# naver/multi-hmr

Hardware: AMD Instinct MI355X
Metric: images/sec (whole node) ViT-L 896x896 bs32 (higher is better)
Workload: dtype f16; 1 GPU; multiHMR_896_L full forward: dinov2_vitl14 896x896, 32 images/GPU, 8 pinned persons/image -> HPH (depth 2) -> SMPL-X LBS; image-sharded x1; global_batch=32, parallelism=dp1 (images)

## Files before the change

multi_hmr_amd/csrc/gemm.hip:

```cpp
#include <stdlib.h>
#include "mhmr_common.h"
#include <string.h>
#include <stdlib.h>
#include "mhmr_internal.h"

namespace {

constexpr int BM = 128, BN = 128, BK = 64;
constexpr int TILE_BYTES = 128 * BK * 2;

template <int DT, int EPI>
__global__ __launch_bounds__(256, 2) void gemm_kernel(const GemmArgs g) {
    typedef typename Op<DT>::T T;
    typedef typename Op<DT>::V8 V8;
    typedef typename Op<DT>::V4 V4;
    extern __shared__ __attribute__((aligned(16))) char smem[];

    const int tid = threadIdx.x, lane = tid & 63;
    const int w = __builtin_amdgcn_readfirstlane(tid >> 6);
    const int hi = lane >> 5, l31 = lane & 31;

    const int nbn = g.N / BN;
    const int bid = xcd_remap(blockIdx.x, gridDim.x);
    const int tn = bid % nbn, tm = bid / nbn;
// ... 131 lines not shown
                    *(f32x4*)op = *(const f32x4*)op + gm * v;
                } else if constexpr (EPI == EPI_PATCH) {
                    if (m < g.Mvalid) {
                        const int b = m / g.Np, n_in = m - b * g.Np;
                        v += *(const f32x4*)(g.pos + (size_t)(1 + n_in) * g.N + n);
                        *(f32x4*)((float*)g.out + ((size_t)b * g.Tp + n_in) * g.ldo + n) = v;
                    }
                } else {
                    *(f32x4*)((float*)g.out + (size_t)m * g.ldo + n) = v;
                }
            }
        }
    } else {
        const int rpi = g.img_rows > 0 ? g.img_rows : g.Tp;
        const int b = m0 / rpi, t0 = m0 - b * rpi;
#pragma unroll
        for (int qj = 0; qj < 2; ++qj) {
            const int n = n0 + 64 * wq_ + 32 * qj + l31;
            const float bv = g.bias ? g.bias[n] : 0.f;
            const int h = n >> 6, d = n & 63;
            T* base = (T*)g.out + ((size_t)(b * g.H + h) * 64 + d) * g.Tp;
#pragma unroll
            for (int pi = 0; pi < 2; ++pi) {
#pragma unroll
                for (int rg = 0; rg < 4; ++rg) {
                    const int t = t0 + 64 * wp_ + 32 * pi + 8 * rg + 4 * hi;
                    const int ts = (t & ~12) | ((t & 4) << 1) | ((t & 8) >> 1);
                    V4 o;
#pragma unroll
                    for (int e = 0; e < 4; ++e) o[e] = (T)(acc[pi][qj][4 * rg + e] + bv);
                    *(V4*)(base + ts) = o;
                }
            }
        }
    }
}

template <int DT>
int launch_dt(const GemmArgs& g, hipStream_t s) {
    const int grid = (g.M / BM) * (g.N / BN);
    const size_t lds = 4 * TILE_BYTES;
#define MHMR_GEMM_CASE(E)                                                                                   \
    case E: {                                                                                               \
        static DeviceOnce once;                                                                             \
        int dev = 0;                                                                                        \
        const int need = once.need(&dev);                                                                   \
        if (need == -2) return MHMR_ERR_BAD_ARG;                                                            \
        if (need >= 0) {                                                                                    \
            hipError_t e = hipFuncSetAttribute((const void*)gemm_kernel<DT, E>, hipFuncAttributeMaxDynamicSharedMemorySize, \
                                               (int)lds);                                                   \
            if (e != hipSuccess) return (int)e;                                                             \
            once.mark(dev);                                                                                 \
        }                                                                                                   \
        hipLaunchKernelGGL((gemm_kernel<DT, E>), dim3(grid), dim3(256), lds, s, g);                         \
        break;                                                                                              \
    }
    switch (g.epi) {
        MHMR_GEMM_CASE(EPI_OP16)
        MHMR_GEMM_CASE(EPI_OP16_GELU)
        MHMR_GEMM_CASE(EPI_OP16_RELU)
        MHMR_GEMM_CASE(EPI_RESID)
        MHMR_GEMM_CASE(EPI_PATCH)
        MHMR_GEMM_CASE(EPI_F32)
        MHMR_GEMM_CASE(EPI_VT)
        MHMR_GEMM_CASE(EPI_OP16_QK)
        default:
            return MHMR_ERR_BAD_ARG;
    }
#undef MHMR_GEMM_CASE
    MHMR_CHECK_LAUNCH();
    return 0;
}

}

int mhmr_cu_count() {
    static std::atomic<int> cus[64];
    int dev = 0;
    if (hipGetDevice(&dev) != hipSuccess) return -1;
    if (dev >= 0 && dev < 64) {
        const int c = cus[dev].load(std::memory_order_relaxed);
        if (c > 0) return c;
    }
    hipDeviceProp_t prop;
    if (hipGetDeviceProperties(&prop, dev) != hipSuccess) return -1;
    if (dev >= 0 && dev < 64) cus[dev].store(prop.multiProcessorCount, std::memory_order_relaxed);
    return prop.multiProcessorCount;
}

namespace {
struct ColGroupEnv {
    int narrow = 2, wide = 2;
    static int lg(int v) { return v <= 0 ? 0 : v == 1 ? 2 : v == 2 ? 1 : v == 4 ? 2 : v == 8 ? 3 : v == 16 ? 4 : v == 32 ? 5 : 0; }
    ColGroupEnv() {
        const char* e = getenv("MHMR_COLGROUP");
        if (!e) return;
        narrow = wide = lg(atoi(e));
        if (const char* c = strchr(e, ',')) wide = lg(atoi(c + 1));
    }
};
}
static const bool g_force_gemm128 = getenv("MHMR_GEMM128") != nullptr;

bool mhmr_splitk_plan(int M, int N, int K, int* ksplit, int* nslices) {
    static const bool on = !(getenv("MHMR_SPLITK") && atoi(getenv("MHMR_SPLITK")) == 0);
    if (!on || g_force_gemm128 || M <= 0 || M % 256 || N % 256 || K % 128) return false;
    if (N > 1024) return false;
    const int ncu = mhmr_cu_count();
    const int tiles = (M / 256) * (N / 256), nt = K / 64;
    if (ncu <= 0 || tiles <= 0) return false;
    int S = ncu / tiles;
    if (S > 8) S = 8;
    if (S > nt / 4) S = nt / 4;
    if (S < 2) return false;
    int ks = (nt + S - 1) / S;
    ks += ks & 1;
    S = (nt + ks - 1) / ks;
    if (S < 2) return false;
    *ksplit = ks;
    *nslices = S;
    return true;
}

int mhmr_launch_gemm(const GemmArgs& g, int dtype, hipStream_t s) {
    if (g.M <= 0 || g.N <= 0 || g.K <= 0 || g.M % BM || g.N % BN || g.K % BK) return MHMR_ERR_BAD_SHAPE;
    if (g.lda % 8 || g.ldw % 8) return MHMR_ERR_BAD_SHAPE;
    if (g.epi == EPI_VT && (g.Tp % 64 || g.N % 64)) return MHMR_ERR_BAD_SHAPE;
    if (g.epi == EPI_VT && (g.img_rows > 0 ? g.img_rows : g.Tp) % BM && (g_force_gemm128 || !mhmr_gemm256_eligible(g))) return MHMR_ERR_BAD_SHAPE;
    if (g.img_rows > 0 && (g.img_rows % BM || g.M % g.img_rows || g.img_stride < g.img_rows || g.epi == EPI_PATCH)) return MHMR_ERR_BAD_SHAPE;
    if (g.a_k > 0 && !g.lo8 && (g.a_k % BK || (g.K != 2 * g.a_k && g.K != 3 * g.a_k) || g.ldw < g.K || (g.K == 3 * g.a_k && g.lda < 2 * g.a_k))) return MHMR_ERR_BAD_SHAPE;
    if (g.epi == EPI_OP16_QK && g.N % 128) return MHMR_ERR_BAD_SHAPE;
    if (g.lo8 && (g_force_gemm128 || !mhmr_gemm256_eligible(g))) return MHMR_ERR_BAD_SHAPE;
    if ((g.x8_off > 0 || g.ldx16 > 0) && !g.x16) return MHMR_ERR_BAD_ARG;
    if (g.ksplit > 0 && (g_force_gemm128 || !mhmr_gemm256_eligible(g))) return MHMR_ERR_BAD_SHAPE;
    if (g.out2 && (g_force_gemm128 || !mhmr_gemm256_eligible(g))) return MHMR_ERR_BAD_SHAPE;
    if (g.n_valid > 0 && g.n_valid != g.N && (g_force_gemm128 || !mhmr_gemm256_eligible(g))) return MHMR_ERR_BAD_SHAPE;
    if (g.x16 || g.pstats || g.rowstats) {
        if (g_force_gemm128 || !mhmr_gemm256_eligible(g)) return MHMR_ERR_BAD_SHAPE;
        if (g.rowstats && g.K < 256) return MHMR_ERR_BAD_SHAPE;
        if (g.rowstats && (g.bias || !g.colsum || !g.fbias || !(g.epi == EPI_OP16_QK || g.epi == EPI_VT || g.epi == EPI_OP16_GELU))) return MHMR_ERR_BAD_ARG;
        if ((g.x16 != nullptr) != (g.pstats != nullptr) || (g.x16 && g.epi != EPI_RESID)) return MHMR_ERR_BAD_ARG;
    }
    prof_begin(PROF_GEMM, s);
    int rc;
    if (!g_force_gemm128 && mhmr_gemm256_eligible(g)) {
        GemmArgs g2 = g;
        static const char* st = getenv("MHMR_STAGGER_PCT");
        const int pct = st ? atoi(st) : (g.img_rows > 0 ? 0 : 100);
        if (g.epi == EPI_RESID && (g.M / 256) * (g.N / 256) >= 1024 && pct > 0)
            g2.stagger_ticks = (int)((g.K / 64 * 1.4 + 18.0) * 25.0 * pct / 100.0);
        static const ColGroupEnv cge;
        const int nbn = g.N / 256;
        g2.colgroup = g.ksplit > 0 ? 0 : nbn >= 16 ? cge.wide : cge.narrow;
        if (g.img_rows > 256) g2.img_magic = (unsigned)((1ull << 32) / (unsigned)(g.img_rows >> 8)) + 1u;
        rc = mhmr_launch_gemm256(g2, dtype, s);
    }
    else rc = dtype == MHMR_DT_F16 ? launch_dt<MHMR_DT_F16>(g, s) : launch_dt<MHMR_DT_BF16>(g, s);
    prof_end(PROF_GEMM, s, 2.0 * g.M * g.N * (g.lo8 ? 2.0 * g.a_k : (double)g.K));
    return rc;
}
```

multi_hmr_amd/csrc/gemm256.hip:

```cpp
#include <type_traits>
#include "mhmr_common.h"
#include "mhmr_internal.h"

namespace {

constexpr int HT = 16384;
constexpr int BUF = 4 * HT;
constexpr int SLOT_P0 = 0, SLOT_P1 = HT, SLOT_Q0 = 2 * HT, SLOT_Q1 = 3 * HT;
constexpr int STAGE_OFF = 2 * BUF;
constexpr int STRIP_OFF = STAGE_OFF + 8 * 2048;
constexpr int LDS_BYTES = 2 * BUF + 8 * 4096;

typedef int v8i_t __attribute__((ext_vector_type(8)));
typedef int v4i_t __attribute__((ext_vector_type(4)));
template <typename V8, bool L8> struct Frag;
template <typename V8> struct Frag<V8, false> {
    V8 k[2];
    __device__ __forceinline__ void set(int ks, V8 x) { k[ks] = x; }
    __device__ __forceinline__ V8 get(int ks) const { return k[ks]; }
    __device__ __forceinline__ v8i_t raw() const {
        return __builtin_shufflevector(__builtin_bit_cast(v4i_t, k[0]), __builtin_bit_cast(v4i_t, k[1]), 0, 1, 2, 3, 4, 5, 6, 7);
    }
};
template <typename V8> struct Frag<V8, true> {
// ... 30 lines not shown
    return v;
}

#ifdef MHMR_GEMM_STAMPS
__device__ unsigned long long* g_gemm_stamps;
__device__ int g_gemm_sametile;
#define GEMM_STAMP(r, i)                                                                                                    \
    do {                                                                                                                    \
        if (g_gemm_stamps && threadIdx.x == 0 && (r) < 64) g_gemm_stamps[((size_t)blockIdx.x * 64 + (r)) * 8 + (i)] = wall_clock64(); \
    } while (0)
#else
#define GEMM_STAMP(r, i)
#endif

template <int DT, int EPI, bool FOLD = false, bool LO8 = false, bool SPLITK = false, bool NMASK = false, bool QKV = false>
__global__ __launch_bounds__(512, 2) void gemm256_kernel(const GemmArgs g) {
    static_assert(!QKV || (EPI == EPI_OP16_QK && !LO8 && !SPLITK && !NMASK), "merged qkv linear: the Q | K epilogue");
    static_assert(!SPLITK || (EPI == EPI_F32 && !FOLD && !LO8), "split-k: fp32 partial tiles only");
    static_assert(!NMASK || ((EPI == EPI_RESID || EPI == EPI_VT) && !LO8 && !SPLITK), "masked output halves: residual and V^T epilogues");
    typedef typename Op<DT>::T T;
    typedef typename Op<DT>::V8 V8;
    typedef typename Op<DT>::V4 V4;
    extern __shared__ __attribute__((aligned(16))) char smem[];

    const int tid = threadIdx.x, lane = tid & 63;
    const int w = __builtin_amdgcn_readfirstlane(tid >> 6);
    const int wp = w >> 2, wq = w & 3;
    const int g4 = lane >> 4, l15 = lane & 15;

    constexpr bool ROWMAJOR = (EPI != EPI_VT);
    constexpr bool FOLDABLE = FOLD;
    static_assert(!FOLD || EPI == EPI_OP16_QK || EPI == EPI_VT || EPI == EPI_OP16_GELU, "consumers of a folded LayerNorm");
    const T* Pm = ROWMAJOR ? (const T*)g.W : (const T*)g.A;
    const T* Qm = ROWMAJOR ? (const T*)g.A : (const T*)g.W;
    const int ldp = ROWMAJOR ? g.ldw : g.lda, ldq = ROWMAJOR ? g.lda : g.ldw;

    const int nbn = g.N / 256, ntiles_real = (g.M / 256) * nbn, ntiles = SPLITK ? ntiles_real * g.nslices : ntiles_real;
    const int G = gridDim.x, b = blockIdx.x;
    const int first = (G & 7) == 0 ? (b & 7) * (G >> 3) + (b >> 3) : b;
    const int cgl = g.colgroup, ncg = cgl > 0 ? nbn >> cgl : 0;
    const bool colgroup = cgl >= 1 && cgl <= 5 && G == 256 && (nbn & ((1 << cgl) - 1)) == 0 && ncg > 1 && ncg <= 8 && (8 % ncg) == 0;

    const int srow = tid >> 3;
    const int schunk = (tid & 7) ^ ((tid >> 4) & 7);
    const int nt = g.K / 64;
    const int nta = g.a_k > 0 ? g.a_k / 64 : nt;
    auto ka = [&](int t) { return (!LO8 && t >= nta) ? t - nta : t; };
    const uint32_t p_lane = (uint32_t)srow * (uint32_t)ldp + (uint32_t)(schunk * 8);
    const uint32_t q_lane = (uint32_t)srow * (uint32_t)ldq + (uint32_t)(schunk * 8);
    auto tile_src = [&](int tix, const T*& pb, const T*& qb, int& p0, int& q0, int& ar, int& bimg, [[maybe_unused]] int& slc) {
        if constexpr (SPLITK) {
            slc = 0;
            while (tix >= ntiles_real) { tix -= ntiles_real; ++slc; }
        }
#ifdef MHMR_GEMM_STAMPS
        if (g_gemm_sametile == 1) tix = 0;
        if (g_gemm_sametile == 2) tix = (int)blockIdx.x;
#endif
        const int tn = tix % nbn, tm = tix / nbn;
        p0 = ROWMAJOR ? tn * 256 : tm * 256;
        q0 = ROWMAJOR ? tm * 256 : tn * 256;
        bimg = 0;
        ar = tm * 256;
        if (g.img_rows > 0) {
            bimg = g.img_magic ? (int)__umulhi((unsigned)tm, g.img_magic) : tm;
            ar = bimg * g.img_stride + (tm - bimg * (g.img_rows >> 8)) * 256;
        }
        pb = Pm + (size_t)(ROWMAJOR ? p0 : ar) * (size_t)ldp;
        qb = Qm + (size_t)(ROWMAJOR ? ar : q0) * (size_t)ldq;
    };
    auto fresh_lane = [&]() {
        int ln = __builtin_amdgcn_mbcnt_hi(~0u, __builtin_amdgcn_mbcnt_lo(~0u, 0u));
        asm volatile("" : "+v"(ln));
        return ln;
    };
    auto dma = [&](const T* base, uint32_t lane_off, int ld, int half, int kt, int lds_off) {
        if constexpr (LO8) {
            const int t2 = w * 64 + fresh_lane();
            lane_off = (uint32_t)(t2 >> 3) * (uint32_t)ld + (uint32_t)((((t2 & 7) ^ ((t2 >> 4) & 7))) * 8);
        }
        const uint32_t o = (lane_off + (uint32_t)(128 * half) * (uint32_t)ld + (uint32_t)(kt * 64)) * (uint32_t)sizeof(T);
        char* d = smem + lds_off + w * 1024;
        glds16((const char*)base + o, d);
        glds16((const char*)base + (o + 64u * (uint32_t)sizeof(T) * (uint32_t)ld), d + 8192);
    };

    const int fsw = l15 >> 1;
    const int pr_off = (64 * wp + l15) * 128, q_off = (32 * wq + l15) * 128;
    int co[2];
#pragma unroll
    for (int ks = 0; ks < 2; ++ks) co[ks] = ((4 * ks + g4) ^ fsw) * 16;

    f32x4 acc[2][2][4][2];
    typedef Frag<V8, LO8> Fr;
    Fr PR[4], QA[2], QB[2];

    auto rdP = [&](int buf, int slot) {
        if constexpr (LO8) {
            const int ln = fresh_lane(), a15 = ln & 15, sw = a15 >> 1, gg = ln >> 4;
            const int po = (64 * wp + a15) * 128, c0 = (gg ^ sw) * 16, c1 = ((4 + gg) ^ sw) * 16;
#pragma unroll
            for (int ps = 0; ps < 4; ++ps)
#pragma unroll
                for (int ks = 0; ks < 2; ++ks) PR[ps].set(ks, *(const V8*)(smem + buf * BUF + slot + po + ps * 2048 + (ks ? c1 : c0)));
        } else {
#pragma unroll
            for (int ps = 0; ps < 4; ++ps)
#pragma unroll
                for (int ks = 0; ks < 2; ++ks) PR[ps].set(ks, *(const V8*)(smem + buf * BUF + slot + pr_off + ps * 2048 + co[ks]));
        }
    };
    auto rdQ = [&](Fr (&Q)[2], int buf, int slot) {
        if constexpr (LO8) {
            const int ln = fresh_lane(), a15 = ln & 15, sw = a15 >> 1, gg = ln >> 4;
            const int qo = (32 * wq + a15) * 128, c0 = (gg ^ sw) * 16, c1 = ((4 + gg) ^ sw) * 16;
#pragma unroll
            for (int qs = 0; qs < 2; ++qs)
#pragma unroll
                for (int ks = 0; ks < 2; ++ks) Q[qs].set(ks, *(const V8*)(smem + buf * BUF + slot + qo + qs * 2048 + (ks ? c1 : c0)));
        } else {
#pragma unroll
            for (int qs = 0; qs < 2; ++qs)
#pragma unroll
                for (int ks = 0; ks < 2; ++ks) Q[qs].set(ks, *(const V8*)(smem + buf * BUF + slot + q_off + qs * 2048 + co[ks]));
        }
    };
    [[maybe_unused]] int w8s = g.w8_scale * 0x01010101, a8s = 0x7F7F7F7F;
    if constexpr (LO8) asm volatile("" : "+v"(w8s), "+v"(a8s));
    auto mma = [&](f32x4 (&c)[4][2], const Fr (&Q)[2], auto lowc) {
        constexpr bool LOW = decltype(lowc)::value;
        __builtin_amdgcn_s_setprio(1);
        if constexpr (LOW) {
#pragma unroll
            for (int ps = 0; ps < 4; ++ps)
#pragma unroll
                for (int qs = 0; qs < 2; ++qs) {
                    if constexpr (ROWMAJOR) mfma_fp8_inplace<0, 1>(c[ps][qs], PR[ps].raw(), Q[qs].raw(), w8s, a8s);
                    else mfma_fp8_inplace<1, 0>(c[ps][qs], PR[ps].raw(), Q[qs].raw(), a8s, w8s);
                }
        } else {
#pragma unroll
            for (int ks = 0; ks < 2; ++ks)
#pragma unroll
                for (int ps = 0; ps < 4; ++ps)
#pragma unroll
                    for (int qs = 0; qs < 2; ++qs) c[ps][qs] = Op<DT>::mfma16(PR[ps].get(ks), Q[qs].get(ks), c[ps][qs]);
        }
        __builtin_amdgcn_s_setprio(0);
    };
#define MHMR_SYNC()                          \
    __builtin_amdgcn_s_barrier();            \
    __builtin_amdgcn_sched_barrier(0)
#define MHMR_WAIT_DMA() asm volatile("s_waitcnt vmcnt(10)" ::: "memory")

    auto acc_init = [&](int h, int j, int qs, int pp0, int qq0) {
        if constexpr (ROWMAJOR) {
#pragma unroll
            for (int ps = 0; ps < 4; ++ps)
                acc[h][j][ps][qs] = g.bias ? *(const f32x4*)(g.bias + pp0 + 128 * h + 64 * wp + 16 * ps + 4 * g4) : (f32x4){0.f, 0.f, 0.f, 0.f};
        } else {
            const float b1 = g.bias ? g.bias[qq0 + 128 * j + 32 * wq + 16 * qs + l15] : 0.f;
#pragma unroll
            for (int ps = 0; ps < 4; ++ps) acc[h][j][ps][qs] = (f32x4){b1, b1, b1, b1};
        }
    };

    const T *p_src, *q_src, *p_nxt, *q_nxt;
    int p0, q0, p0n, q0n, ar, arn, bimg, bimgn;
    [[maybe_unused]] int sl = 0, sln = 0;
    if (first >= ntiles) return;
    if (g.stagger_ticks > 0) {
        const uint64_t t0 = wall_clock64(), dl = (uint64_t)g.stagger_ticks * (uint64_t)(first * 4 / G);
        while (wall_clock64() - t0 < dl) __builtin_amdgcn_s_sleep(32);
    }
    const int full = ntiles / G, nmine = full + (b < ntiles - full * G ? 1 : 0);
    auto tile_of = [&](int r) {
        if (r >= full) return full * G + b;
        if (colgroup) {
            const int x = b & 7, slot = b >> 3;
            const int row = r * (G / nbn) + (x / ncg) * (32 >> cgl) + (slot >> cgl), col = ((x % ncg) << cgl) + (slot & ((1 << cgl) - 1));
            return row * nbn + col;
        }
        return first + r * G;
    };
    tile_src(tile_of(0), p_src, q_src, p0, q0, ar, bimg, sl);
    int kb = 0, kbn = 0, ntc = nt;
    if constexpr (SPLITK) { kb = sl * g.ksplit; ntc = nt - kb < g.ksplit ? nt - kb : g.ksplit; }

    {
        const int k0p = !SPLITK ? 0 : ROWMAJOR ? kb : ka(kb), k1p = !SPLITK ? 1 : ROWMAJOR ? kb + 1 : ka(kb + 1);
        const int k0q = !SPLITK ? 0 : ROWMAJOR ? ka(kb) : kb, k1q = !SPLITK ? 1 : ROWMAJOR ? ka(kb + 1) : kb + 1;
        dma(q_src, q_lane, ldq, 0, k0q, SLOT_Q0);
        dma(p_src, p_lane, ldp, 0, k0p, SLOT_P0);
        dma(q_src, q_lane, ldq, 1, k0q, SLOT_Q1);
        dma(p_src, p_lane, ldp, 1, k0p, SLOT_P1);
        dma(q_src, q_lane, ldq, 1, k1q, BUF + SLOT_Q1);
        dma(p_src, p_lane, ldp, 0, k1p, BUF + SLOT_P0);
        dma(q_src, q_lane, ldq, 0, k1q, BUF + SLOT_Q0);
    }
#pragma unroll
    for (int a = 0; a < 8; ++a) acc_init(a >> 2, (a >> 1) & 1, a & 1, p0, q0);
    asm volatile("s_waitcnt vmcnt(0)" ::: "memory");
    MHMR_SYNC();

    for (int r = 0; r < nmine; ++r) {
        GEMM_STAMP(r, 0);
        rdQ(QA, 0, SLOT_Q0);
        if (wp == 1) { MHMR_SYNC(); }
        const bool has_next = r + 1 < nmine;
        if (has_next) tile_src(tile_of(r + 1), p_nxt, q_nxt, p0n, q0n, arn, bimgn, sln);
        else { p_nxt = p_src; q_nxt = q_src; p0n = p0; q0n = q0; arn = ar; bimgn = bimg; sln = sl; }
        if constexpr (SPLITK) kbn = sln * g.ksplit;
        auto kpair = [&](int t, auto lowc) {
            const bool wrap = t + 2 >= ntc;
            const T* p2 = wrap ? p_nxt : p_src;
            const T* q2 = wrap ? q_nxt : q_src;
            const int t1 = kb + t + 1, t2 = wrap ? (has_next ? kbn : kb + ntc - 1) : kb + t + 2, t3 = wrap ? (has_next ? kbn + 1 : kb + ntc - 1) : kb + t + 3;
            const int t1p = ROWMAJOR ? t1 : ka(t1), t2p = ROWMAJOR ? t2 : ka(t2), t3p = ROWMAJOR ? t3 : ka(t3);
            const int t2q = ROWMAJOR ? ka(t2) : t2, t3q = ROWMAJOR ? ka(t3) : t3;
            if constexpr (FOLDABLE) {
                if (wrap && w < 4) {
                    const int nbase = ROWMAJOR ? p0 : q0;
                    const float* sp = w == 0 ? g.colsum + nbase : w == 1 ? g.fbias + nbase : g.rowstats + 2 * (size_t)ar + (w - 2) * 256;
                    const int ln = __builtin_amdgcn_mbcnt_hi(~0u, __builtin_amdgcn_mbcnt_lo(~0u, 0u));
                    glds16(sp + ln * 4, smem + STRIP_OFF + w * 1024);
                }
            }
            rdP(0, SLOT_P0);
            dma(p_src, p_lane, ldp, 1, t1p, BUF + SLOT_P1); MHMR_WAIT_DMA();
            MHMR_SYNC(); mma(acc[0][0], QA, lowc); MHMR_SYNC();
            rdQ(QB, 0, SLOT_Q1);
            dma(q2, q_lane, ldq, 0, t2q, SLOT_Q0); MHMR_WAIT_DMA();
            MHMR_SYNC(); mma(acc[0][1], QB, lowc); MHMR_SYNC();
            rdP(0, SLOT_P1);
            dma(p2, p_lane, ldp, 0, t2p, SLOT_P0); MHMR_WAIT_DMA();
            MHMR_SYNC(); mma(acc[1][1], QB, lowc); MHMR_SYNC();
            rdQ(QB, 1, SLOT_Q1);
            dma(q2, q_lane, ldq, 1, t2q, SLOT_Q1); MHMR_WAIT_DMA();
            MHMR_SYNC(); mma(acc[1][0], QA, lowc); MHMR_SYNC();
            rdP(1, SLOT_P0);
            dma(p2, p_lane, ldp, 1, t2p, SLOT_P1); MHMR_WAIT_DMA();
            MHMR_SYNC(); mma(acc[0][1], QB, lowc); MHMR_SYNC();
            rdQ(QA, 1, SLOT_Q0);
            dma(q2, q_lane, ldq, 1, t3q, BUF + SLOT_Q1); MHMR_WAIT_DMA();
            MHMR_SYNC(); mma(acc[0][0], QA, lowc); MHMR_SYNC();
            rdP(1, SLOT_P1);
            dma(p2, p_lane, ldp, 0, t3p, BUF + SLOT_P0); MHMR_WAIT_DMA();
            MHMR_SYNC(); mma(acc[1][0], QA, lowc); MHMR_SYNC();
            if (!wrap) rdQ(QA, 0, SLOT_Q0);
            dma(q2, q_lane, ldq, 0, t3q, BUF + SLOT_Q0); MHMR_WAIT_DMA();
            MHMR_SYNC(); mma(acc[1][1], QB, lowc); MHMR_SYNC();
        };
        for (int t = 0; t < (LO8 ? nta : ntc); t += 2) kpair(t, std::false_type{});
        if constexpr (LO8)
            for (int t = nta; t < nt; t += 2) kpair(t, std::true_type{});

        GEMM_STAMP(r, 1);
        if (wp == 0) { MHMR_SYNC(); }
        GEMM_STAMP(r, 2);
        char* wl = smem + STAGE_OFF + w * 4096;
        constexpr bool RELANE = FOLD || EPI == EPI_RESID;
        int lane_e = 0;
        if constexpr (RELANE) {
            lane_e = __builtin_amdgcn_mbcnt_hi(~0u, __builtin_amdgcn_mbcnt_lo(~0u, 0u));
            asm volatile("" : "+v"(lane_e));
        }
        const int lane_outer = lane, l15_outer = l15, g4_outer = g4;
        {
        const int lane = RELANE ? lane_e : lane_outer;
        const int l15 = RELANE ? (lane_e & 15) : l15_outer, g4 = RELANE ? (lane_e >> 4) : g4_outer;
        constexpr bool OUT16 = (EPI == EPI_OP16 || EPI == EPI_OP16_GELU || EPI == EPI_OP16_RELU || EPI == EPI_VT || EPI == EPI_OP16_QK);
        if constexpr (EPI == EPI_RESID) {
            constexpr int RD = 1;
            const int c = lane & 15;
            const uint32_t off0 = ((uint32_t)(ar + 32 * wq + (lane >> 4)) * (uint32_t)g.ldo + (uint32_t)(p0 + 64 * wp + 4 * c)) * 4u;
            const uint32_t rstep = (uint32_t)g.ldo * 16u;
            [[maybe_unused]] const int nvalid = NMASK ? g.n_valid : g.N;
            [[maybe_unused]] const bool dead1 = NMASK && p0 + 128 >= nvalid;
            auto live = [&](int sidx) { return !NMASK || !(dead1 && (sidx >> 2) == 1); };
            auto rptr = [&](int sidx, int it) {
                const int h = sidx >> 2, j = (sidx >> 1) & 1, qs = sidx & 1;
                const uint32_t hoff = NMASK ? (live(sidx) ? (uint32_t)(512 * h) : 0u) : (uint32_t)(512 * h);
                const uint32_t off = off0 + (uint32_t)(32 * j + 4 * qs + it) * rstep + hoff;
                return (f32x4*)((char*)g.out + off);
            };
            f32x4 r[8][4];
#pragma unroll
            for (int sidx = 0; sidx < RD; ++sidx)
#pragma unroll
                for (int it = 0; it < 4; ++it) r[sidx][it] = *rptr(sidx, it);
            f32x4 gm[2];
#pragma unroll
            for (int h = 0; h < 2; ++h) gm[h] = *(const f32x4*)(g.gamma + p0 + 128 * h + 64 * wp + 4 * c);
#pragma unroll
            for (int sidx = 0; sidx < 8; ++sidx) {
                const int h = sidx >> 2, j = (sidx >> 1) & 1, qs = sidx & 1;
                if (sidx + RD < 8) {
#pragma unroll
                    for (int it = 0; it < 4; ++it) r[sidx + RD][it] = *rptr(sidx + RD, it);
                }
#pragma unroll
                for (int ps = 0; ps < 4; ++ps) *(f32x4*)(wl + l15 * 256 + (((4 * ps + g4) ^ l15) * 16)) = acc[h][j][ps][qs];
                acc_init(h, j, qs, p0n, q0n);
                if (!live(sidx)) continue;
#pragma unroll
                for (int it = 0; it < 4; ++it) {
                    const int row = 4 * it + (lane >> 4);
                    const f32x4 v = *(const f32x4*)(wl + row * 256 + ((c ^ row) * 16));
                    const f32x4 nv = r[sidx][it] + gm[h] * v;
                    f32x4* rp = rptr(sidx, it);
                    *rp = nv;
                    if (g.x16 != nullptr) {
                        const uint32_t off = (uint32_t)((char*)rp - (char*)g.out);
                        V4 o;
#pragma unroll
                        for (int e = 0; e < 4; ++e) o[e] = (T)nv[e];
                        if (g.ldx16 > 0) {
                            const uint32_t prow = (uint32_t)(ar + 32 * wq + (lane >> 4)) + (uint32_t)(4 * (32 * j + 4 * qs + it));
                            const uint32_t pcol = (uint32_t)(p0 + 64 * wp + 4 * c + 128 * h);
                            char* xrow = (char*)g.x16 + (size_t)prow * ((uint32_t)g.ldx16 * 2u);
                            *(V4*)(xrow + pcol * 2u) = o;
                            if (g.x8_off > 0) *(uint32_t*)(xrow + (uint32_t)g.x8_off + pcol) = pack_bf8x4(nv[0], nv[1], nv[2], nv[3]);
                        } else {
                            *(V4*)((char*)g.x16 + (off >> 1)) = o;
                        }
                        float s1 = (nv[0] + nv[1]) + (nv[2] + nv[3]);
                        float s2 = (nv[0] * nv[0] + nv[1] * nv[1]) + (nv[2] * nv[2] + nv[3] * nv[3]);
                        s1 = row16_sum(s1);
                        s2 = row16_sum(s2);
                        if (c == 0) {
                            const int prow = ar + 128 * j + 32 * wq + 16 * qs + row;
                            const int slot = (p0 + 128 * h + 64 * wp) >> 6;
                            *(f32x2*)(g.pstats + ((size_t)prow * (nvalid >> 6) + slot) * 2) = (f32x2){s1, s2};
                        }
                    }
                }
            }
        } else {
        constexpr bool fold = FOLD;
        [[maybe_unused]] const float* strip = (const float*)(smem + STRIP_OFF);
        constexpr int NPASS = FOLDABLE ? 2 : 1;
        if constexpr (FOLDABLE) wl = smem + STAGE_OFF + w * 2048;
#pragma unroll
        for (int h = 0; h < 2; ++h) {
#pragma unroll
            for (int j = 0; j < 2; ++j) {
                const int pb = p0 + 128 * h + 64 * wp;
                const int qb = q0 + 128 * j + 32 * wq;
                const int qphys = ar + 128 * j + 32 * wq;
                if constexpr (NMASK && EPI == EPI_VT) {
                    if (q0 + 128 * j >= g.n_valid) {
                        acc_init(h, j, 0, p0n, q0n);
                        acc_init(h, j, 1, p0n, q0n);
                        continue;
                    }
                }
                if constexpr (OUT16) {
                    const float qscale = (EPI == EPI_OP16_QK && pb < (QKV ? g.qcols : (g.N >> 1))) ? MHMR_ATTN_QSCALE : 1.f;
#pragma unroll
                    for (int qh = 0; qh < NPASS; ++qh) {
                        [[maybe_unused]] float qa2[2] = {0.f, 0.f}, qb2[2] = {0.f, 0.f};
                        if constexpr (FOLDABLE) {
                            if (fold) {
                                const int qpos = 128 * j + 32 * wq + 16 * qh + l15;
                                if constexpr (ROWMAJOR) { const f32x2 mr = *(const f32x2*)(strip + 512 + 2 * qpos); qa2[qh] = mr[1]; qb2[qh] = -mr[0] * mr[1]; }
                                else { qa2[qh] = strip[qpos]; qb2[qh] = strip[256 + qpos]; }
                            }
                        }
#pragma unroll
                        for (int ps = 0; ps < 4; ++ps) {
                            const int pc = 16 * ps + 4 * g4;
                            [[maybe_unused]] f32x4 pa4 = {0.f, 0.f, 0.f, 0.f}, pb4 = {0.f, 0.f, 0.f, 0.f};
                            if constexpr (FOLDABLE) {
                                if (fold) {
                                    const int ppos = 128 * h + 64 * wp + pc;
                                    if constexpr (ROWMAJOR) { pa4 = *(const f32x4*)(strip + ppos); pb4 = *(const f32x4*)(strip + 256 + ppos); }
                                    else {
                                        const f32x4 m0 = *(const f32x4*)(strip + 512 + 2 * ppos), m1 = *(const f32x4*)(strip + 512 + 2 * ppos + 4);
                                        pa4 = (f32x4){m0[1], m0[3], m1[1], m1[3]};
                                        pb4 = (f32x4){-m0[0] * m0[1], -m0[2] * m0[3], -m1[0] * m1[1], -m1[2] * m1[3]};
                                    }
                                }
                            }
                            const int gs = ((g4 & 1) << 1) | (g4 >> 1);
                            const int pos = ROWMAJOR ? pc : 16 * ps + 4 * gs;
#pragma unroll
                            for (int qs = FOLDABLE ? qh : 0; qs < (FOLDABLE ? qh + 1 : 2); ++qs) {
                                const int qr = FOLDABLE ? l15 : 16 * qs + l15;
                                V4 o;
#pragma unroll
                                for (int e = 0; e < 4; ++e) {
                                    float v = acc[h][j][ps][qs][e];
                                    if constexpr (FOLDABLE) {
                                        if (fold) {
                                            if constexpr (ROWMAJOR) v = __builtin_fmaf(v, qa2[qs], __builtin_fmaf(qb2[qs], pa4[e], pb4[e]));
                                            else v = __builtin_fmaf(v, pa4[e], __builtin_fmaf(pb4[e], qa2[qs], qb2[qs]));
                                        }
                                    }
                                    if constexpr (EPI == EPI_OP16_GELU) v = gelu_fast(v);
                                    if constexpr (EPI == EPI_OP16_RELU) v = fmaxf(v, 0.f);
                                    if constexpr (EPI == EPI_OP16_QK) v *= qscale;
                                    o[e] = (T)v;
                                }
                                *(V4*)(wl + qr * 128 + (((pos >> 2) ^ ((qr & 7) << 1)) * 8)) = o;
                            }
                        }
                        if constexpr (FOLDABLE) acc_init(h, j, qh, p0n, q0n);
                        else { acc_init(h, j, 0, p0n, q0n); acc_init(h, j, 1, p0n, q0n); }
#pragma unroll
                        for (int it = 0; it < (FOLDABLE ? 2 : 4); ++it) {
                            const int srow = 8 * it + (lane >> 3), c16 = lane & 7;
                            const int row = (FOLDABLE ? 16 * qh : 0) + srow;
                            const u32x4 v = *(const u32x4*)(wl + srow * 128 + ((c16 ^ (srow & 7)) * 16));
                            if constexpr (ROWMAJOR && QKV) {
                                const bool second = pb >= g.split_col;
                                T* ob = second ? (T*)g.out2 : (T*)g.out;
                                const int ld = second ? g.ldo2 : g.ldo, col = second ? pb - g.split_col : pb;
                                *(u32x4*)(ob + (size_t)(qphys + row) * ld + col + c16 * 8) = v;
                            } else if constexpr (ROWMAJOR) {
                                *(u32x4*)((T*)g.out + (size_t)(qphys + row) * g.ldo + pb + c16 * 8) = v;
                            } else {
                                const int n = qb + row, bi = g.img_rows > 0 ? bimg : pb / g.Tp, tl = pb - bi * (g.img_rows > 0 ? g.img_rows : g.Tp);
                                *(u32x4*)((T*)g.out + ((size_t)(bi * g.H + (n >> 6)) * 64 + (n & 63)) * g.Tp + tl + c16 * 8) = v;
                            }
                        }
                    }
                } else {
                    const int c = lane & 15;
                    const int n = pb + 4 * c;
#pragma unroll
                    for (int qs = 0; qs < 2; ++qs) {
#pragma unroll
                        for (int ps = 0; ps < 4; ++ps) {
                            const int ch = 4 * ps + g4;
                            *(f32x4*)(wl + l15 * 256 + ((ch ^ l15) * 16)) = acc[h][j][ps][qs];
                        }
                        acc_init(h, j, qs, p0n, q0n);
#pragma unroll
                        for (int it = 0; it < 4; ++it) {
                            const int row = 4 * it + (lane >> 4);
                            f32x4 v = *(const f32x4*)(wl + row * 256 + ((c ^ row) * 16));
                            const int m = qb + 16 * qs + row;
                            if constexpr (EPI == EPI_PATCH) {
                                if (m < g.Mvalid) {
                                    const int bi = m / g.Np, n_in = m - bi * g.Np;
                                    v += *(const f32x4*)(g.pos + (size_t)(1 + n_in) * g.N + n);
                                    *(f32x4*)((float*)g.out + ((size_t)bi * g.Tp + n_in) * g.ldo + n) = v;
                                }
                            } else {
                                if constexpr (SPLITK) *(f32x4*)((float*)g.out + ((size_t)sl * g.M + (size_t)(qphys + 16 * qs + row)) * g.ldo + n) = v;
                                else *(f32x4*)((float*)g.out + (size_t)(qphys + 16 * qs + row) * g.ldo + n) = v;
                            }
                        }
                    }
                }
            }
        }
        }
        }
        GEMM_STAMP(r, 3);
        asm volatile("s_waitcnt vmcnt(0)" ::: "memory");
        GEMM_STAMP(r, 4);
        p_src = p_nxt; q_src = q_nxt; p0 = p0n; q0 = q0n; ar = arn; bimg = bimgn;
        if constexpr (SPLITK) { sl = sln; kb = kbn; ntc = nt - kb < g.ksplit ? nt - kb : g.ksplit; }
    }
#undef MHMR_SYNC
#undef MHMR_WAIT_DMA
}

#ifdef MHMR_GEMM_STAMPS
}
extern "C" __attribute__((visibility("default"))) int mhmr_debug_gemm_stamps(void* p) { return (int)hipMemcpyToSymbol(HIP_SYMBOL(g_gemm_stamps), &p, sizeof(p)); }
extern "C" __attribute__((visibility("default"))) int mhmr_debug_gemm_sametile(int v) { return (int)hipMemcpyToSymbol(HIP_SYMBOL(g_gemm_sametile), &v, sizeof(v)); }
namespace {
#endif

template <int DT>
int launch256_dt(const GemmArgs& g, hipStream_t s) {
    const int ntiles = (g.M / 256) * (g.N / 256) * (g.ksplit > 0 ? g.nslices : 1);
    const int ncu = mhmr_cu_count();
    if (ncu <= 0) return MHMR_ERR_BAD_ARG;
    const int grid = ntiles < ncu ? ntiles : ncu;
#define MHMR_GEMM_LAUNCH11(E, F, L8, SK, NM, QV)                                                               \
    {                                                                                                          \
        static DeviceOnce once;                                                                                \
        int dev = 0;                                                                                           \
        const int need = once.need(&dev);                                                                      \
        if (need == -2) return MHMR_ERR_BAD_ARG;                                                               \
        if (need >= 0) {                                                                                       \
            hipError_t e = hipFuncSetAttribute((const void*)gemm256_kernel<DT, E, F, L8, SK, NM, QV>, hipFuncAttributeMaxDynamicSharedMemorySize, \
                                               LDS_BYTES);                                                     \
            if (e != hipSuccess) return (int)e;                                                                \
            once.mark(dev);                                                                                    \
        }                                                                                                      \
        mhmr_launch_kernel(gemm256_kernel<DT, E, F, L8, SK, NM, QV>, dim3(grid), dim3(512), LDS_BYTES, s, g);  \
    }
#define MHMR_GEMM_LAUNCH10(E, F, L8, SK, NM) MHMR_GEMM_LAUNCH11(E, F, L8, SK, NM, false)
#define MHMR_GEMM_LAUNCH9(E, F, L8, SK) MHMR_GEMM_LAUNCH10(E, F, L8, SK, false)
#define MHMR_GEMM_LAUNCH8(E, F, L8) MHMR_GEMM_LAUNCH9(E, F, L8, false)
#define MHMR_GEMM_LAUNCH(E, F) MHMR_GEMM_LAUNCH8(E, F, false)
#define MHMR_GEMM_CASE(E) \
    case E: MHMR_GEMM_LAUNCH(E, false) break;
    if (g.ksplit > 0) {
        MHMR_GEMM_LAUNCH9(EPI_F32, false, false, true)
        MHMR_CHECK_LAUNCH();
        return 0;
    }
    if (g.out2) {
        if (g.epi != EPI_OP16_QK) return MHMR_ERR_BAD_ARG;
        if (g.rowstats) MHMR_GEMM_LAUNCH11(EPI_OP16_QK, true, false, false, false, true)
        else MHMR_GEMM_LAUNCH11(EPI_OP16_QK, false, false, false, false, true)
        MHMR_CHECK_LAUNCH();
        return 0;
    }
    if (g.n_valid > 0 && g.n_valid != g.N) {
        if (g.epi == EPI_RESID && !g.rowstats) MHMR_GEMM_LAUNCH10(EPI_RESID, false, false, false, true)
        else if (g.epi == EPI_VT && g.rowstats) MHMR_GEMM_LAUNCH10(EPI_VT, true, false, false, true)
        else if (g.epi == EPI_VT) MHMR_GEMM_LAUNCH10(EPI_VT, false, false, false, true)
        else return MHMR_ERR_BAD_ARG;
        MHMR_CHECK_LAUNCH();
        return 0;
    }
    if (g.lo8) {
        if (g.epi == EPI_VT && g.rowstats != nullptr) MHMR_GEMM_LAUNCH8(EPI_VT, true, true)
        else if (g.epi == EPI_VT) MHMR_GEMM_LAUNCH8(EPI_VT, false, true)
        else if (g.epi == EPI_RESID) MHMR_GEMM_LAUNCH8(EPI_RESID, false, true)
        else return MHMR_ERR_BAD_ARG;
        MHMR_CHECK_LAUNCH();
        return 0;
    }
    if (g.rowstats != nullptr) {
        switch (g.epi) {
            case EPI_OP16_GELU: MHMR_GEMM_LAUNCH(EPI_OP16_GELU, true) break;
            case EPI_VT: MHMR_GEMM_LAUNCH(EPI_VT, true) break;
            case EPI_OP16_QK: MHMR_GEMM_LAUNCH(EPI_OP16_QK, true) break;
            default: return MHMR_ERR_BAD_ARG;
        }
        MHMR_CHECK_LAUNCH();
        return 0;
    }
    switch (g.epi) {
        MHMR_GEMM_CASE(EPI_OP16)
        MHMR_GEMM_CASE(EPI_OP16_GELU)
        MHMR_GEMM_CASE(EPI_OP16_RELU)
        MHMR_GEMM_CASE(EPI_RESID)
        MHMR_GEMM_CASE(EPI_PATCH)
        MHMR_GEMM_CASE(EPI_F32)
        MHMR_GEMM_CASE(EPI_VT)
        MHMR_GEMM_CASE(EPI_OP16_QK)
        default:
            return MHMR_ERR_BAD_ARG;
    }
#undef MHMR_GEMM_CASE
#undef MHMR_GEMM_LAUNCH
#undef MHMR_GEMM_LAUNCH8
#undef MHMR_GEMM_LAUNCH9
#undef MHMR_GEMM_LAUNCH10
#undef MHMR_GEMM_LAUNCH11
    MHMR_CHECK_LAUNCH();
    return 0;
}

}

bool mhmr_gemm256_eligible(const GemmArgs& g) {
    const uint64_t mphys = g.img_rows > 0 ? (uint64_t)(g.M / g.img_rows) * (uint64_t)g.img_stride : (uint64_t)g.M;
    if (g.epi == EPI_RESID && mphys * (uint64_t)g.ldo * 4u >= (1ull << 32)) return false;
    if (g.img_rows > 0 && (g.img_rows % 256 || g.M % g.img_rows || g.epi == EPI_PATCH)) return false;
    if (g.lo8) {
        if (g.a_k <= 0 || g.a_k % 256 || g.K != g.a_k + g.a_k / 2 || g.lda < g.K || g.ldw < g.K || !(g.epi == EPI_VT || g.epi == EPI_RESID)) return false;
    } else if (g.a_k > 0 && (g.a_k % 128 || (g.K != 2 * g.a_k && g.K != 3 * g.a_k))) return false;
    if (g.lda >= (1 << 22) || g.ldw >= (1 << 22)) return false;
    if (g.n_valid > 0 && g.n_valid != g.N) {
        if (g.n_valid % 128 || g.n_valid > g.N || g.N - g.n_valid != 128 || g.lo8 || g.ksplit > 0 || !(g.epi == EPI_RESID || g.epi == EPI_VT)) return false;
    }
    if (g.out2) {
        if (g.epi != EPI_OP16_QK || g.split_col <= 0 || g.split_col % 64 || g.split_col >= g.N || g.qcols < 0 || g.qcols % 64 || g.qcols > g.split_col ||
            g.ldo2 < g.N - g.split_col || g.lo8 || g.ksplit > 0 || g.n_valid > 0)
            return false;
    }
    if (g.ksplit > 0) {
        const int nt = g.K / 64;
        if (g.epi != EPI_F32 || g.bias || g.lo8 || g.img_rows > 0 || g.ksplit % 2 || g.nslices < 2 || g.nslices > 16 ||
            (g.nslices - 1) * g.ksplit >= nt || g.nslices * g.ksplit < nt || g.ldo != g.N)
            return false;
    }
    return g.M % 256 == 0 && g.N % 256 == 0 && g.K % 128 == 0 && (g.epi != EPI_VT || g.Tp % 64 == 0);
}

int mhmr_launch_gemm256(const GemmArgs& g, int dtype, hipStream_t s) {
    return dtype == MHMR_DT_F16 ? launch256_dt<MHMR_DT_F16>(g, s) : launch256_dt<MHMR_DT_BF16>(g, s);
}
```

multi_hmr_amd/csrc/mhmr_internal.h:

```cpp
#pragma once
#include <hip/hip_runtime.h>
#include <stdint.h>
#include "../../include/mhmr.h"

enum GemmEpilogue {
    EPI_OP16 = 0,
    EPI_OP16_GELU = 1,
    EPI_OP16_RELU = 2,
    EPI_RESID = 3,
    EPI_PATCH = 4,
    EPI_F32 = 5,
    EPI_VT = 6,
    EPI_OP16_QK = 7,
};

struct GemmArgs {
    const void* A; int lda;
    const void* W; int ldw;
    int M, N, K;
    const float* bias;
    const float* gamma;
    void* out; int ldo;
    const float* pos;
    int Np, Tp, H, Mvalid;
    int epi;
    int stagger_ticks = 0;
    int img_rows = 0, img_stride = 0;
    unsigned img_magic = 0;
    int a_k = 0;
    int lo8 = 0;
    int w8_scale = 127;
    int ldx16 = 0, x8_off = 0;
    int colgroup = 0;
    void* x16 = nullptr;
    float* pstats = nullptr;
    const float* rowstats = nullptr;
    const float* colsum = nullptr;
    const float* fbias = nullptr;
    int ksplit = 0, nslices = 0;
    int n_valid = 0;
    void* out2 = nullptr;
    int ldo2 = 0, split_col = 0, qcols = 0;
};

__host__ __device__ inline long long mhmr_phys_row(int m, int img_rows, int img_stride) {
    return img_rows > 0 ? (long long)(m / img_rows) * img_stride + (m % img_rows) : (long long)m;
}

#include <atomic>
struct DeviceOnce {
    std::atomic<uint64_t> done{0};
    int need(int* dev_out) {
        int dev = 0;
        if (hipGetDevice(&dev) != hipSuccess) return -2;
        *dev_out = dev;
        if (dev >= 0 && dev < 64 && ((done.load(std::memory_order_relaxed) >> dev) & 1ull)) return -1;
        return dev;
    }
    void mark(int dev) { if (dev >= 0 && dev < 64) done.fetch_or(1ull << dev, std::memory_order_relaxed); }
};
extern thread_local int g_mhmr_anyorder;
#include <hip/hip_ext.h>
template <typename F, typename... Args>
inline void mhmr_launch_kernel(F kernel, dim3 grid, dim3 block, size_t lds, hipStream_t s, Args... args) {
    if (g_mhmr_anyorder) hipExtLaunchKernelGGL(kernel, grid, block, (uint32_t)lds, s, nullptr, nullptr, hipExtAnyOrderLaunch, args...);
    else hipLaunchKernelGGL(kernel, grid, block, lds, s, args...);
}

struct ClsArgs {
    const void* A = nullptr; long long a_stride = 0;
    const void* W = nullptr; int ldw = 0;
    int B = 0, N = 0, K = 0, a_k = 0;
    const float* bias = nullptr; const float* gamma = nullptr;
    void* out = nullptr; long long o_stride = 0;
    int n_base = 0, C = 0;
    void* vt = nullptr; int H = 0, Tp = 0, vcol = 0;
    const float* rowstats = nullptr; long long rs_stride = 0; const float* colsum = nullptr; const float* fbias = nullptr;
    void* x16 = nullptr; long long x_stride = 0;
    float* cls_pstats = nullptr; int cls_nblk = 0, cls_C = 0; float cls_eps = 1e-6f;
    const float* st_pstats = nullptr; float* st_rowstats = nullptr; int st_blocks = 0, st_B = 0, st_N = 0, st_Tp = 0, st_C = 0;
};
enum { CLS_QKV = 0, CLS_RESID = 1, CLS_GELU = 2 };

enum ProfKind { PROF_GEMM = 0, PROF_ATTN = 1, PROF_LBS = 2, PROF_KINDS = 3 };

void prof_begin(int kind, hipStream_t s);
void prof_end(int kind, hipStream_t s, double work);

int mhmr_launch_gemm(const GemmArgs& g, int dtype, hipStream_t s);
int mhmr_cu_count();
bool mhmr_splitk_plan(int M, int N, int K, int* ksplit, int* nslices);

bool mhmr_gemm256_eligible(const GemmArgs& g);
int mhmr_launch_gemm256(const GemmArgs& g, int dtype, hipStream_t s);

int mhmr_launch_attention(const void* qk, const void* vt, void* out, int B, int T, int Tp, int C, int H, int dtype, int* flags, hipStream_t s,
                          int ldo = 0, int o8 = 0);
int mhmr_launch_attention_ex(const void* qk, const void* vt, void* out, int B, int T, int Tp, int C, int H, int dtype, float limit_log2,
                             int variant, int* flags, hipStream_t s);
int mhmr_attention_flag_count_impl(int B, int Tp, int H);

int mhmr_launch_attention_f32(const float* qkv, void* out, int B, int T, int Tp, int C, int H, int dtype, hipStream_t s);

int mhmr_launch_im2col(const float* x, void* a, int B, int S, int G, int Kp, int dtype, hipStream_t s);
int mhmr_launch_im2col_pair(const float* x, void* a, int B, int S, int G, int Kp, int dtype, hipStream_t s);
int mhmr_launch_init_rows(float* resid, const float* cls_pos0, int B, int T, int Tp, int C, hipStream_t s);
int mhmr_launch_layernorm(const float* in, const float* w, const float* b, void* out16, int rows, int C, float eps, int dtype, hipStream_t s);
int mhmr_launch_layernorm_pitch(const float* in, const float* w, const float* b, void* out16, int ld16, int o8, int rows, int C, float eps,
                                int dtype, hipStream_t s);
int mhmr_launch_layernorm_pair(const float* in, const float* w, const float* b, void* out16, int rows, int C, float eps, int dtype,
                               hipStream_t s);
int mhmr_launch_gelu_pair(const float* in, void* out, long long M, int N, int dtype, hipStream_t s);
int mhmr_launch_vt_transpose(const void* v, int ldv, void* vt, int B, int Tp, int H, int dtype, hipStream_t s);
int mhmr_launch_splitk_resid(const float* part, int nslices, int rows, int C, const float* bias, const float* gamma, float* resid, void* x16,
                             int ldx, float* rowstats, float eps, int dtype, hipStream_t s);
int mhmr_launch_ln_stats(const float* pstats, const float* resid, float* rowstats, int B, int N, int Tp, int C, float eps, hipStream_t s);
int mhmr_launch_final_norm(const float* resid, const float* w, const float* b, void* ctx16, int ldctx, float* feat32, int B, int Np, int Tp,
                           int C, float eps, int dtype, hipStream_t s);

int mhmr_launch_cls_linear(const ClsArgs& a, int epi, int dtype, hipStream_t s);

int mhmr_launch_linear_f32(const float* X, int ldx, const int* row_idx, const float* W, int ldw, const float* bias, const float* R, int ldr,
                           float* Y, int ldy, int M, int N, int K, int act, hipStream_t s);
int mhmr_launch_layernorm_f32(const float* in, const float* w, const float* b, float* out, int rows, int C, float eps, hipStream_t s);
int mhmr_launch_scores(const void* hid, int ld, const float* w2, const float* b2, float* scores, int rows, int C, int dtype, hipStream_t s);
int mhmr_launch_detect_count(const float* scores, int B, int G, int nms_kernel, float thr, int* counts, hipStream_t s);
int mhmr_launch_detect_write(const float* scores, int B, int G, int nms_kernel, float thr, const int* base, int* det_b, int* det_y, int* det_x,
                             float* det_score, int cap, hipStream_t s);
int mhmr_launch_person_groups(const int* counts, const int* det_b, int P, int B, int cap, int* base, int* gstart, int ngcap, int* chunks,
                              int nccap, int* info, hipStream_t s);
int mhmr_launch_camera_embed(const float* Kmat, const float* freq, int B, int G, int patch, float* zK, void* ctx16, int Kc, int C, int dtype,
                             int nbands, hipStream_t s);
int mhmr_launch_hph_inputs(const float* feat32, const float* zK, const int* det_b, const int* det_y, const int* det_x, const float* cq_x,
                           const float* cq_y, const float* cv_x, const float* cv_y, const float* init_tail, int ntail, float* zc, float* token,
                           int Ktok, void* ctx16, int Kc, int* det_row, int P, int G, int C, int dtype, const int* nvalid, int cam_dim,
                           hipStream_t s);
int mhmr_launch_hph_self_attn(const float* qkv, const int* gstart, float* out, int ngroups, int nmax, int heads, hipStream_t s);
int mhmr_launch_hph_cross_attn(const float* q, const float* kv, const int* chunks, int nchunks, float* out, int heads, int N, hipStream_t s);
int mhmr_launch_hph_decode(const float* dec, int ldd, int nb, const float* Kmat, const int* det_b, float fn, int nearness, float* rotmat,
                           float* rotvec, float* betas, float* expr, float* dist_pp, float* dist, int P, hipStream_t s);
int mhmr_launch_loc(const float* offset, const int* det_y, const int* det_x, int patch, float* loc, int P, hipStream_t s);
```

Before: 235.7 images/s.

## Overlap epilogue stores with next tile's mainloop in folded GEMM256

In the persistent GEMM256 kernel's folded path, the full vmcnt(0) drain at the end of each tile's epilogue is replaced by a seam flag. The first k-pair of the next tile then waits with a vmcnt threshold raised by the number of outstanding epilogue stores, so output stores overlap the next tile's loads and MFMAs instead of stalling the wave. Folded accumulators are also initialised to zero rather than loading bias. An env var MHMR_GEMM_DRAIN restores the old drain. The approach depends on exact store counts per wave, checked by a static_assert, and a wrong count could produce a race.

```diff
diff --git a/multi_hmr_amd/csrc/gemm.hip b/multi_hmr_amd/csrc/gemm.hip
--- a/multi_hmr_amd/csrc/gemm.hip
+++ b/multi_hmr_amd/csrc/gemm.hip
@@ -307,6 +307,7 @@
         static const ColGroupEnv cge;
         const int nbn = g.N / 256;
         g2.colgroup = g.ksplit > 0 ? 0 : nbn >= 16 ? cge.wide : cge.narrow;
+        { const char* dr = getenv("MHMR_GEMM_DRAIN"); g2.seam_drain = dr && atoi(dr) != 0; }
         if (g.img_rows > 256) g2.img_magic = (unsigned)((1ull << 32) / (unsigned)(g.img_rows >> 8)) + 1u;
         rc = mhmr_launch_gemm256(g2, dtype, s);
     }
diff --git a/multi_hmr_amd/csrc/gemm256.hip b/multi_hmr_amd/csrc/gemm256.hip
--- a/multi_hmr_amd/csrc/gemm256.hip
+++ b/multi_hmr_amd/csrc/gemm256.hip
@@ -206,9 +206,30 @@
     __builtin_amdgcn_s_barrier();            \
     __builtin_amdgcn_sched_barrier(0)
 #define MHMR_WAIT_DMA() asm volatile("s_waitcnt vmcnt(10)" ::: "memory")
+    constexpr bool SEAM = FOLD;
+    constexpr int SEAM_STORES = 16;
+    [[maybe_unused]] int seam = 0;
+    auto wait_dma_seam = [&](int sw) {
+        if constexpr (SEAM && NMASK) {
+            asm volatile("s_waitcnt vmcnt(%1)\n\ts_cmp_eq_u32 %0, 1\n\ts_cbranch_scc1 1f\n\ts_waitcnt vmcnt(%2)\n\ts_cmp_eq_u32 %0, 2\n\ts_cbranch_scc1 1f\n\t"
+                         "s_waitcnt vmcnt(10)\n1:" ::"s"(sw), "n"(10 + SEAM_STORES), "n"(10 + SEAM_STORES / 2) : "memory", "scc");
+        } else if constexpr (SEAM) {
+            asm volatile("s_waitcnt vmcnt(%1)\n\ts_cmp_eq_u32 %0, 1\n\ts_cbranch_scc1 1f\n\ts_waitcnt vmcnt(10)\n1:" ::"s"(sw), "n"(10 + SEAM_STORES) : "memory", "scc");
+        } else {
+            MHMR_WAIT_DMA();
+        }
+    };
+#define MHMR_WAIT_DMA_SEAM()                                        \
+    do {                                                            \
+        if constexpr (decltype(lowc)::value) MHMR_WAIT_DMA();       \
+        else wait_dma_seam(sw);                                     \
+    } while (0)
 
     auto acc_init = [&](int h, int j, int qs, int pp0, int qq0) {
-        if constexpr (ROWMAJOR) {
+        if constexpr (FOLD) {
+#pragma unroll
+            for (int ps = 0; ps < 4; ++ps) acc[h][j][ps][qs] = (f32x4){0.f, 0.f, 0.f, 0.f};
+        } else if constexpr (ROWMAJOR) {
 #pragma unroll
             for (int ps = 0; ps < 4; ++ps)
                 acc[h][j][ps][qs] = g.bias ? *(const f32x4*)(g.bias + pp0 + 128 * h + 64 * wp + 16 * ps + 4 * g4) : (f32x4){0.f, 0.f, 0.f, 0.f};
@@ -272,6 +293,12 @@
             const int t1 = kb + t + 1, t2 = wrap ? (has_next ? kbn : kb + ntc - 1) : kb + t + 2, t3 = wrap ? (has_next ? kbn + 1 : kb + ntc - 1) : kb + t + 3;
             const int t1p = ROWMAJOR ? t1 : ka(t1), t2p = ROWMAJOR ? t2 : ka(t2), t3p = ROWMAJOR ? t3 : ka(t3);
             const int t2q = ROWMAJOR ? ka(t2) : t2, t3q = ROWMAJOR ? ka(t3) : t3;
+            [[maybe_unused]] int sw = 0;
+            if constexpr (SEAM && !decltype(lowc)::value) {
+                sw = seam;
+                seam = 0;
+                asm volatile("" : "+s"(seam));
+            }
             if constexpr (FOLDABLE) {
                 if (wrap && w < 4) {
                     const int nbase = ROWMAJOR ? p0 : q0;
@@ -281,20 +308,23 @@
                 }
             }
             rdP(0, SLOT_P0);
-            dma(p_src, p_lane, ldp, 1, t1p, BUF + SLOT_P1); MHMR_WAIT_DMA();
+            dma(p_src, p_lane, ldp, 1, t1p, BUF + SLOT_P1); MHMR_WAIT_DMA_SEAM();
             MHMR_SYNC(); mma(acc[0][0], QA, lowc); MHMR_SYNC();
             rdQ(QB, 0, SLOT_Q1);
-            dma(q2, q_lane, ldq, 0, t2q, SLOT_Q0); MHMR_WAIT_DMA();
+            dma(q2, q_lane, ldq, 0, t2q, SLOT_Q0); MHMR_WAIT_DMA_SEAM();
             MHMR_SYNC(); mma(acc[0][1], QB, lowc); MHMR_SYNC();
             rdP(0, SLOT_P1);
-            dma(p2, p_lane, ldp, 0, t2p, SLOT_P0); MHMR_WAIT_DMA();
+            dma(p2, p_lane, ldp, 0, t2p, SLOT_P0); MHMR_WAIT_DMA_SEAM();
             MHMR_SYNC(); mma(acc[1][1], QB, lowc); MHMR_SYNC();
             rdQ(QB, 1, SLOT_Q1);
-            dma(q2, q_lane, ldq, 1, t2q, SLOT_Q1); MHMR_WAIT_DMA();
+            dma(q2, q_lane, ldq, 1, t2q, SLOT_Q1); MHMR_WAIT_DMA_SEAM();
             MHMR_SYNC(); mma(acc[1][0], QA, lowc); MHMR_SYNC();
             rdP(1, SLOT_P0);
-            dma(p2, p_lane, ldp, 1, t2p, SLOT_P1); MHMR_WAIT_DMA();
+            dma(p2, p_lane, ldp, 1, t2p, SLOT_P1); MHMR_WAIT_DMA_SEAM();
             MHMR_SYNC(); mma(acc[0][1], QB, lowc); MHMR_SYNC();
+#ifdef MHMR_GEMM_STAMPS
+            if (t == 0) GEMM_STAMP(r, 5);
+#endif
             rdQ(QA, 1, SLOT_Q0);
             dma(q2, q_lane, ldq, 1, t3q, BUF + SLOT_Q1); MHMR_WAIT_DMA();
             MHMR_SYNC(); mma(acc[0][0], QA, lowc); MHMR_SYNC();
@@ -394,6 +424,8 @@
         constexpr bool fold = FOLD;
         [[maybe_unused]] const float* strip = (const float*)(smem + STRIP_OFF);
         constexpr int NPASS = FOLDABLE ? 2 : 1;
+        constexpr int NIT = FOLDABLE ? 2 : 4;
+        static_assert(!SEAM || (OUT16 && 2 * 2 * NPASS * NIT == SEAM_STORES), "SEAM: the store instructions a tile's epilogue leaves in a wave's queue");
         if constexpr (FOLDABLE) wl = smem + STAGE_OFF + w * 2048;
 #pragma unroll
         for (int h = 0; h < 2; ++h) {
@@ -462,7 +494,7 @@
                         if constexpr (FOLDABLE) acc_init(h, j, qh, p0n, q0n);
                         else { acc_init(h, j, 0, p0n, q0n); acc_init(h, j, 1, p0n, q0n); }
 #pragma unroll
-                        for (int it = 0; it < (FOLDABLE ? 2 : 4); ++it) {
+                        for (int it = 0; it < NIT; ++it) {
                             const int srow = 8 * it + (lane >> 3), c16 = lane & 7;
                             const int row = (FOLDABLE ? 16 * qh : 0) + srow;
                             const u32x4 v = *(const u32x4*)(wl + srow * 128 + ((c16 ^ (srow & 7)) * 16));
@@ -513,13 +545,23 @@
         }
         }
         GEMM_STAMP(r, 3);
-        asm volatile("s_waitcnt vmcnt(0)" ::: "memory");
+        if constexpr (SEAM) {
+            if (g.seam_drain) {
+                asm volatile("s_waitcnt vmcnt(0)" ::: "memory");
+                seam = 0;
+            } else {
+                seam = (NMASK && EPI == EPI_VT && q0 + 128 >= g.n_valid) ? 2 : 1;
+            }
+        } else {
+            asm volatile("s_waitcnt vmcnt(0)" ::: "memory");
+        }
         GEMM_STAMP(r, 4);
         p_src = p_nxt; q_src = q_nxt; p0 = p0n; q0 = q0n; ar = arn; bimg = bimgn;
         if constexpr (SPLITK) { sl = sln; kb = kbn; ntc = nt - kb < g.ksplit ? nt - kb : g.ksplit; }
     }
 #undef MHMR_SYNC
 #undef MHMR_WAIT_DMA
+#undef MHMR_WAIT_DMA_SEAM
 }
 
 #ifdef MHMR_GEMM_STAMPS
diff --git a/multi_hmr_amd/csrc/mhmr_internal.h b/multi_hmr_amd/csrc/mhmr_internal.h
--- a/multi_hmr_amd/csrc/mhmr_internal.h
+++ b/multi_hmr_amd/csrc/mhmr_internal.h
@@ -31,6 +31,7 @@
     int lo8 = 0;
     int w8_scale = 127;
     int ldx16 = 0, x8_off = 0;
+    int seam_drain = 0;
     int colgroup = 0;
     void* x16 = nullptr;
     float* pstats = nullptr;
```

Result: no change. 234.3 images/s (-0.6%).
